# leejeongho3214/LightHand

Hardware: AMD Instinct MI355X
Metric: images/sec/GPU (256×256, bs=64) train+infer; EPE/AUC parity (higher is better)
Workload: dtype bf16; 1 GPU; SimpleBaseline-ResNet50 256x256 training step (fwd + JointsMSELoss + argmax decode + bwd + Adam), batch 64/GPU, 21 joints, random init (seed 9001), hipGraph replay; global_batch=64, parallelism=dp1

## Files before the change

### lighthand_amd/csrc/conv3x3_direct_kernel.h

```cpp
#pragma once
#include "igemm_ring_kernel.h"
#include "igemm_wave_epilogue.h"
#include <stdlib.h>

#pragma clang diagnostic push
#pragma clang diagnostic ignored "-Winline-asm"
__device__ __forceinline__ void d3_lds_dma16(const unsigned char* src, unsigned lds) {
    asm volatile("s_mov_b32 m0, %1\n\ts_nop 0\n\tglobal_load_lds_dwordx4 %0, off" ::"v"(src), "s"(lds) : "memory", "m0");
}
#pragma clang diagnostic pop

template <typename T, int C, bool STATS, bool GATE = false>
__device__ __forceinline__ void conv3x3_direct_body(const IgemmArgs& p, unsigned char* smem, const int b) {
    constexpr int ES = sizeof(T);
    static_assert(ES == 2 && (C == 32 || C == 64), "16-bit element types, 32 or 64 input channels per tap");
    constexpr int BM = 64, TH = 16, TW = 16, PH = TH + 2, PW = TW + 2;
    constexpr int NWAVE = 8;
    constexpr int ROWB = C * ES;
    constexpr int SL = ROWB / 16;
    constexpr int PPI = 1024 / ROWB;
    constexpr int KS = C / 32;
    constexpr int WBYTES = 9 * BM * ROWB;
    constexpr int NPIX = PH * PW;
    constexpr int NPI = (NPIX + PPI - 1) / PPI;
    constexpr int NPW = (NPI + NWAVE - 1) / NWAVE;
    constexpr int PATCH = NPIX * ROWB;
    constexpr int PT = TH / NWAVE;
    constexpr int RS = 64 * ES + 8;
    constexpr int STG = PT * 16 * RS;
    constexpr bool ALIAS = NWAVE * STG <= PATCH;
    constexpr int OFF_PATCH = WBYTES, OFF_STG = WBYTES + 2 * PATCH, OFF_CST = OFF_STG + (ALIAS ? 0 : NWAVE * STG);
    constexpr int NWT = WBYTES / 1024;

    const int tid = threadIdx.x, lane = tid & 63;
    const int wave = __builtin_amdgcn_readfirstlane(tid >> 6);
    const int q = lane >> 4, pl = lane & 15;
    const unsigned lds_base = (unsigned)(size_t)(__attribute__((address_space(3))) unsigned char*)smem;
    const int CB = p.pw_cb, G = p.pw_g;
    const int cblk = (b >> 3) % CB;
// ... 54 lines not shown
        flive = tile < ntile;
        const int tt = flive ? tile : 0;
        const int n = tt / (ty_n * tx_n), rem = tt - n * (ty_n * tx_n);
        fy0 = (rem / tx_n) * TH - 1;
        fx0 = (rem % tx_n) * TW - 1;
        fbase = p.in + n * img_stride;
    };
    auto fetch_piece = [&](int j, int buf) {
        const int iy = fy0 + ppy[j], ix = fx0 + ppx[j];
        const bool ok = flive & ((unsigned)iy < (unsigned)p.hi) & ((unsigned)ix < (unsigned)p.wi);
        const unsigned char* src = ok ? fbase + iy * row_stride + (long)ix * pix_stride + pch[j] : p.zero;
        const unsigned dst = lds_base + OFF_PATCH + buf * PATCH + (NWAVE * j + wave) * 1024;
        if (!(LH_ABL & 4) && ppy[j] >= 0) d3_lds_dma16(src, dst);
    };
    unsigned aoff[KS];
#pragma unroll
    for (int kk = 0; kk < KS; ++kk) aoff[kk] = pl * ROWB + ((((SL == 8 ? 4 * kk : 0) + q) ^ fswz(pl)) << 4);

    float s1[STATS ? 1 : 1][8], s2[STATS ? 1 : 1][8], s3[1][8];
#pragma unroll
    for (int e = 0; e < 8; ++e) s1[0][e] = s2[0][e] = 0.f;
    const float* cst = reinterpret_cast<const float*>(smem + OFF_CST);

    int t = g;
    tile_origin(t);
#pragma unroll
    for (int j = 0; j < NPW; ++j) fetch_piece(j, 0);
    asm volatile("s_waitcnt vmcnt(0)" ::: "memory");
    int buf = 0;
    for (; t < ntile; t += G, buf ^= 1) {
        asm volatile("s_waitcnt lgkmcnt(0)" ::: "memory");
        __builtin_amdgcn_s_barrier();
        asm volatile("" ::: "memory");
        tile_origin(t + G);
        const unsigned char* patch = smem + OFF_PATCH + buf * PATCH;
        f32x4 acc[4][PT];
#pragma unroll
        for (int i = 0; i < 4; ++i)
#pragma unroll
            for (int j = 0; j < PT; ++j) acc[i][j] = f32x4{0.f, 0.f, 0.f, 0.f};
        constexpr int NSTEP = 9 * KS;
        static_assert(NPW <= NSTEP, "one patch piece per MFMA step");
        uint4 A[2][4], B[2][PT];
        auto rd = [&](int step, uint4 (&a)[4], uint4 (&bb)[PT]) {
            const int tap = step / KS, kk = step % KS;
            const int dy = p.dh[tap] + 1, dx = p.dw[tap] + 1;
#pragma unroll
            for (int i = 0; i < 4; ++i) {
                if (LH_ABL & 2) a[i] = uint4{aoff[kk] + i, 3u, 5u, 7u};
                else a[i] = *reinterpret_cast<const uint4*>(smem + tap * (BM * ROWB) + i * 16 * ROWB + aoff[kk]);
            }
#pragma unroll
            for (int j = 0; j < PT; ++j) {
                const int pp = (PT * wave + j + dy) * PW + dx + pl;
                const unsigned off = pp * ROWB + ((((SL == 8 ? 4 * kk : 0) + q) ^ fswz(pp)) << 4);
                if (LH_ABL & 2) bb[j] = uint4{off, 1u, 2u, 3u};
                else bb[j] = *reinterpret_cast<const uint4*>(patch + off);
            }
// ... 9 lines not shown
#pragma unroll
                for (int j = 0; j < PT; ++j) {
                    if (LH_ABL & 1) acc[i][j][0] += __builtin_bit_cast(float, A[step & 1][i].x ^ B[step & 1][j].x);
                    else MmaR<T>::run(A[step & 1][i], B[step & 1][j], acc[i][j]);
                }
            __builtin_amdgcn_sched_barrier(0);
        }
        if (LH_ABL & 8) {
            float z = 0.f;
#pragma unroll
            for (int i = 0; i < 4; ++i)
#pragma unroll
                for (int j = 0; j < PT; ++j) z += acc[i][j][0] + acc[i][j][1] + acc[i][j][2] + acc[i][j][3];
            if (z == 123.456f) p.out[0] = 1;
            asm volatile("s_waitcnt vmcnt(0)" ::: "memory");
            continue;
        }
        if (ALIAS) {
            asm volatile("s_waitcnt lgkmcnt(0)" ::: "memory");
            __builtin_amdgcn_s_barrier();
            asm volatile("" ::: "memory");
        }
        unsigned char* stg = (ALIAS ? smem + OFF_PATCH + buf * PATCH : smem + OFF_STG) + wave * STG;
        const int n = t / (ty_n * tx_n), rem = t - n * (ty_n * tx_n);
        const int oy0 = (rem / tx_n) * TH + PT * wave, ox0 = (rem % tx_n) * TW;
        wave_epilogue<T, BM, PT, STATS, (GATE ? 1 : 0)>(p, acc, stg, cst, cblk, lane, [&](int row) {
            const int y = oy0 + (row >> 4), x = ox0 + (row & 15);
            return (y < H && x < W) ? ((long)n * H + y) * W + x : -1L;
        }, s1, s2, s3);
        asm volatile("s_waitcnt vmcnt(%0)" ::"n"(2 * PT) : "memory");
    }
    if constexpr (STATS) {
        asm volatile("s_waitcnt vmcnt(0)" ::: "memory");
        __syncthreads();
        wave_stats_row<BM, NWAVE>(s1, s2, reinterpret_cast<float*>(smem), p.stats ? p.stats + (long)g * 2 * p.cout : nullptr, cblk, p.cout, tid);
    }
}

template <typename T, int C, bool STATS, bool GATE = false>
__global__ __launch_bounds__(512, 2) void conv3x3_direct_kernel(const IgemmArgs p) {
    extern __shared__ __attribute__((aligned(16))) unsigned char smem[];
    conv3x3_direct_body<T, C, STATS, GATE>(p, smem, blockIdx.x);
}

static inline int lh_d3_lds_bytes(int c) {
    const int patch = 18 * 18 * c * 2, stg = 8 * 2 * 16 * 136;
    return 9 * 64 * c * 2 + 2 * patch + (stg <= patch ? 0 : stg) + 2 * 64 * 4;
}

static inline void lh_d3_grid(int c, int n, int h, int w, int cout, int* G, int* CB) {
    const int cb = (cout + 63) / 64;
    const int occ = lh_d3_lds_bytes(c) <= 80 * 1024 ? 2 : 1;
// ... 33 lines not shown
```

### lighthand_amd/csrc/igemm_epilogue.h

```cpp
#pragma once
#include "common.h"
#include "igemm_args.h"

#ifndef LH_ABL
#define LH_ABL 0
#endif

template <typename T, int BM, int BP, bool HEAD> constexpr int lh_epi_lds_bytes() {
    return BP * (BM * (int)sizeof(T) + 8) + (HEAD ? 32 * (BM * (int)sizeof(T) + 16) : 0) + 3 * BM * 4;
}

template <int BM, int NT>
__device__ __forceinline__ void igemm_epilogue_consts(const IgemmArgs& p, float* cst, int c0, int tid) {
    const int cmax = p.cout - 1;
    for (int c = tid; c < BM; c += NT) {
        const int gc = c0 + c, gk = gc < cmax ? gc : cmax;
        const bool ok = gc < p.cout;
        const float b = p.bias ? p.bias[gk] : 0.f, sc = p.scale ? p.scale[gk] : 1.f, sh = p.scale ? p.shift[gk] : 0.f;
        float bv = (p.bias && ok) ? b : 0.f, sv = 1.f;
        if (p.scale) {
            sv = ok ? sc : 1.f;
            bv = bv * sv + (ok ? sh : 0.f);
        }
        cst[c] = sv;
        cst[BM + c] = bv;
    }
}

template <int NR, int EPC, bool GATE> struct EpilogueGate {
    uint4 xd[NR];
    unsigned gbits[NR];
    float gmean[EPC], ginv[EPC], gsc[EPC], gsh[EPC];
};
template <int NR, int EPC> struct EpilogueGate<NR, EPC, false> {};

template <typename T, int BM, int BP, int WC, int WP, bool GATE = false>
__device__ __forceinline__ void igemm_epilogue(const IgemmArgs& p, unsigned char* smem, f32x4 (&acc)[BM / WC / 16][BP / WP / 16],
                                               int pblk, int cblk, int tid, int lane, int wc, int wp, int hw,
                                               int ooh, int oow, float* stats) {
    constexpr int ES = sizeof(T);
    constexpr int EPC = 16 / ES;
    constexpr int TC = BM / WC, TP = BP / WP;
    constexpr int CT = TC / 16, PT = TP / 16;
    constexpr int RS = BM * ES + 8;
    if (LH_ABL & 8) { if (acc[0][0][0] == 123.456f) p.out[0] = 1; return; }
    if (LH_ABL & 32) {
        float t = 0.f;
#pragma unroll
        for (int i = 0; i < BM / WC / 16; ++i)
#pragma unroll
            for (int j = 0; j < BP / WP / 16; ++j) t += acc[i][j][0] + acc[i][j][1] + acc[i][j][2] + acc[i][j][3];
        if (t == 123.456f) p.out[0] = 1;
        return;
    }
    __syncthreads();
    float* cst = reinterpret_cast<float*>(smem + BP * RS);
    const bool affine = p.bias || p.scale;
    if (affine) {
        igemm_epilogue_consts<BM, 64 * WC * WP>(p, cst, cblk * BM, tid);
        __syncthreads();
    }
    const int q = lane >> 4, pl = lane & 15;
#pragma unroll
    for (int i = 0; i < CT; ++i) {
        const int col = wc * TC + i * 16 + q * 4;
        float4 s4 = float4{1.f, 1.f, 1.f, 1.f}, b4 = float4{0.f, 0.f, 0.f, 0.f};
        if (affine) {
            s4 = *reinterpret_cast<const float4*>(cst + col);
            b4 = *reinterpret_cast<const float4*>(cst + BM + col);
        }
        const float sv[4] = {s4.x, s4.y, s4.z, s4.w}, bv[4] = {b4.x, b4.y, b4.z, b4.w};
#pragma unroll
        for (int j = 0; j < PT; ++j) {
            const int pr = wp * TP + j * 16 + pl;
            T* dst = reinterpret_cast<T*>(smem + pr * RS + col * ES);
            if constexpr (ES == 4) {
                reinterpret_cast<float2*>(dst)[0] = float2{acc[i][j][0] * sv[0] + bv[0], acc[i][j][1] * sv[1] + bv[1]};
                reinterpret_cast<float2*>(dst)[1] = float2{acc[i][j][2] * sv[2] + bv[2], acc[i][j][3] * sv[3] + bv[3]};
            } else {
                union { uint2 u; T e[4]; } pk;
#pragma unroll
                for (int r = 0; r < 4; ++r) pk.e[r] = from_f<T>(acc[i][j][r] * sv[r] + bv[r]);
                *reinterpret_cast<uint2*>(dst) = pk.u;
            }
        }
    }
    __syncthreads();

    constexpr int CH = BM * ES / 16;
    constexpr int NT = 64 * WC * WP;
    constexpr int RPP = NT / CH;
    const int chunk = tid % CH, r0 = tid / CH;
    const int col0 = cblk * BM + chunk * EPC;
    const bool col_ok = col0 < p.cout;
    float s1[EPC], s2[EPC];
#pragma unroll
    for (int e = 0; e < EPC; ++e) s1[e] = s2[e] = 0.f;

    const bool dense = p.osh == 1 && p.osw == 1 && p.OH == p.ho && p.OW == p.wo && ooh == 0 && oow == 0;
    int m = pblk * BP + r0;
    int pn = 0, pa = 0, pb = 0;
    const int qa = RPP / p.wo, step_b = RPP - qa * p.wo, step_n = qa / p.ho, step_a = qa - step_n * p.ho;
    if (!dense) {
        pn = m / hw;
        const int rem = m - pn * hw;
        pa = rem / p.wo;
        pb = rem - pa * p.wo;
    }
    constexpr int NR = BP / RPP;
    static_assert(BP % RPP == 0, "rows per thread");
    int opx[NR];
    uint4 ad[NR];
    unsigned mbits[NR];
    EpilogueGate<NR, EPC, GATE> gt;
    if constexpr (GATE) {
#pragma unroll
        for (int e = 0; e < EPC; ++e) {
            const int gk = col0 + e < p.cout ? col0 + e : p.cout - 1;
            gt.gmean[e] = p.gmean[gk]; gt.ginv[e] = p.ginv[gk];
            gt.gsc[e] = p.gmask ? 0.f : p.gscale[gk]; gt.gsh[e] = p.gmask ? 0.f : p.gshift[gk];
        }
    }
#pragma unroll
    for (int k = 0; k < NR; ++k, m += RPP) {
        int opix = m;
        if (!dense) {
            opix = (pn * p.OH + pa * p.osh + ooh) * p.OW + pb * p.osw + oow;
            pb += step_b; pa += step_a; pn += step_n;
            if (pb >= p.wo) { pb -= p.wo; ++pa; }
            if (pa >= p.ho) { pa -= p.ho; ++pn; }
        }
        opx[k] = (m < p.M && col_ok) ? opix : -1;
        ad[k] = uint4{0u, 0u, 0u, 0u};
        mbits[k] = 0xffu;
        if (p.addend) {
            const bool ok = opx[k] >= 0;
            const long eoff = (long)((unsigned long)(unsigned)(ok ? opx[k] : 0) * (unsigned)p.out_pix_stride) + col0;
            ad[k] = *reinterpret_cast<const uint4*>(ok ? p.addend + eoff * ES : p.zero);
            if (p.addend_mask) mbits[k] = *(ok ? p.addend_mask + eoff / EPC : p.zero);
        }
        if constexpr (GATE) {
            gt.gbits[k] = 0xffu;
            const bool ok = opx[k] >= 0;
            const long eoff = (long)((unsigned long)(unsigned)(ok ? opx[k] : 0) * (unsigned)p.out_pix_stride) + col0;
            gt.xd[k] = *reinterpret_cast<const uint4*>(ok ? p.gx + eoff * ES : p.zero);
            if (p.gmask) gt.gbits[k] = *(ok ? p.gmask + eoff / EPC : p.zero);
        }
    }
#pragma unroll
    for (int k = 0; k < NR; ++k) {
        if (opx[k] < 0) continue;
        const int pr = r0 + k * RPP;
        const long eoff = (long)((unsigned long)(unsigned)opx[k] * (unsigned)p.out_pix_stride) + col0;
        const unsigned char* src = smem + pr * RS + chunk * 16;
        const uint2 lo = *reinterpret_cast<const uint2*>(src);
        const uint2 hi = *reinterpret_cast<const uint2*>(src + 8);
        uint4 u = uint4{lo.x, lo.y, hi.x, hi.y};
        if (p.addend || p.relu) {
            float v[EPC];
            unpack16<T>(u, v);
            if (p.addend) {
                float av[EPC];
                unpack16<T>(ad[k], av);
                if (p.addend_mask) {
#pragma unroll
                    for (int e = 0; e < EPC; ++e) av[e] = ((mbits[k] >> e) & 1u) ? av[e] : 0.f;
                }
#pragma unroll
                for (int e = 0; e < EPC; ++e) v[e] += av[e];
            }
            if (p.relu) {
// ... 133 lines not shown
```

### lighthand_amd/csrc/igemm_pw_kernel.h

```cpp
#pragma once
#include "igemm_ring_kernel.h"
#include "igemm_wave_epilogue.h"
#include <stdlib.h>

template <typename T, int BM, int KC, int PT, bool STATS, int GATE = 0>
__global__ __launch_bounds__(256, 2) void igemm_pw_kernel(const IgemmArgs p) {
    static_assert(!GATE || STATS, "the gate leaves its sums in the statistics row");
    constexpr bool DB = KC <= 256 && !(BM == 256 && KC >= 128) && (2 * PT * (KC / 32) * 4 + (BM / 16) * PT * 4 + (STATS ? (BM / 64) * 16 : 0)) <= 176;
    extern __shared__ __attribute__((aligned(16))) unsigned char smem[];
    constexpr int ES = sizeof(T);
    static_assert(ES == 2, "16-bit element types only");
    constexpr int EPC = 8;
    constexpr int CT = BM / 16;
    constexpr int KS = KC / 32;
    constexpr int NSP = KC / 64;
    constexpr int SPB = BM * 128;
    constexpr int PANEL = NSP * SPB;
    constexpr int SUBW = 64;
    constexpr int NSB = BM / SUBW;
    constexpr int RS = SUBW * ES + 8;
    constexpr int STG = PT * 16 * RS;
    constexpr int CST = PANEL + 4 * STG;
    constexpr int NI = PANEL / 1024;
    static_assert(NI % 4 == 0 && NI / 4 <= 60, "panel fill: instructions per wave");

    const int tid = threadIdx.x, lane = tid & 63;
    const int wave = __builtin_amdgcn_readfirstlane(tid >> 6);
    const int q = lane >> 4, pl = lane & 15;
    const int CB = p.pw_cb, G = p.pw_g;
    const int b = blockIdx.x;
    const int cblk = (b >> 3) % CB;
// ... 61 lines not shown
        }
    };
    int t = g * 4 + wave;
    uint4 B0[PT][KS], B1[DB ? PT : 1][DB ? KS : 1];
    loadB(t, B0);
    asm volatile("s_waitcnt vmcnt(0)" ::: "memory");
    __syncthreads();

    const unsigned aoff0 = pl * 128 + (((0 + q) ^ ((pl >> 1) & 7)) << 4);
    const unsigned aoff1 = pl * 128 + (((4 + q) ^ ((pl >> 1) & 7)) << 4);
    unsigned char* stg = smem + PANEL + wave * STG;
    const float* cst = reinterpret_cast<const float*>(smem + CST);

    float s1[STATS ? NSB : 1][EPC], s2[STATS ? NSB : 1][EPC], s3[GATE == 2 ? NSB : 1][EPC];
#pragma unroll
    for (int i = 0; i < (STATS ? NSB : 1); ++i)
#pragma unroll
        for (int e = 0; e < EPC; ++e) s1[i][e] = s2[i][e] = 0.f;
#pragma unroll
    for (int i = 0; i < (GATE == 2 ? NSB : 1); ++i)
#pragma unroll
        for (int e = 0; e < EPC; ++e) s3[i][e] = 0.f;

    auto tilework = [&](const int t, uint4 (&Bf)[PT][KS], auto&& prefetch) {
        f32x4 acc[CT][PT];
#pragma unroll
        for (int i = 0; i < CT; ++i)
#pragma unroll
            for (int j = 0; j < PT; ++j) acc[i][j] = f32x4{0.f, 0.f, 0.f, 0.f};
        constexpr int NG = KS * (CT / 4);
        uint4 A[2][4];
        auto readA = [&](auto Gc, uint4 (&dst)[4]) {
            constexpr int grp = decltype(Gc)::value;
            constexpr int kk = grp / (CT / 4), i0 = (grp % (CT / 4)) * 4;
#pragma unroll
            for (int u = 0; u < 4; ++u)
                if (LH_ABL & 2) dst[u] = uint4{aoff0 + u, aoff1, 5u, 7u};
                else dst[u] = *reinterpret_cast<const uint4*>(smem + (kk >> 1) * SPB + (i0 + u) * 2048 + ((kk & 1) ? aoff1 : aoff0));
        };
        readA(ic<0>{}, A[0]);
        static_for<0, NG>([&](auto Gc) {
            constexpr int grp = decltype(Gc)::value;
            constexpr int kk = grp / (CT / 4), i0 = (grp % (CT / 4)) * 4;
            if constexpr (grp + 1 < NG) readA(ic<grp + 1>{}, A[(grp + 1) & 1]);
            __builtin_amdgcn_sched_barrier(0);
#pragma unroll
            for (int u = 0; u < 4; ++u)
#pragma unroll
                for (int j = 0; j < PT; ++j) {
                    if (LH_ABL & 1) acc[i0 + u][j][0] += __builtin_bit_cast(float, A[grp & 1][u].x ^ Bf[j][kk].x);
                    else MmaR<T>::run(A[grp & 1][u], Bf[j][kk], acc[i0 + u][j]);
                }
            __builtin_amdgcn_sched_barrier(0);
        });
        prefetch();

        if (LH_ABL & 8) {
            float z = 0.f;
#pragma unroll
            for (int i = 0; i < CT; ++i)
#pragma unroll
                for (int j = 0; j < PT; ++j) z += acc[i][j][0] + acc[i][j][1] + acc[i][j][2] + acc[i][j][3];
            if (z == 123.456f) p.out[0] = 1;
            return;
        }
        const int m0 = t * PT * 16;
        wave_epilogue<T, BM, PT, STATS, GATE>(p, acc, stg, cst, cblk, lane, [&](int row) { const int m = m0 + row; return m < M ? (long)m : -1L; }, s1, s2, s3);
    };
    if constexpr (DB) {
        while (t < ntile) {
            loadB(t + tstride, B1);
            tilework(t, B0, [] {});
            t += tstride;
            if (t >= ntile) break;
            loadB(t + tstride, B0);
            tilework(t, B1, [] {});
            t += tstride;
        }
    } else {
        for (; t < ntile; t += tstride) tilework(t, B0, [&] { loadB(t + tstride, B0); });
    }

    if constexpr (STATS) {
        __syncthreads();
        wave_stats_row<BM, 4>(s1, s2, reinterpret_cast<float*>(smem), p.stats ? p.stats + (long)g * 2 * p.cout : nullptr, cblk, p.cout, tid);
        if constexpr (GATE == 2) {
            __syncthreads();
            wave_stats_row<BM, 4>(s1, s3, reinterpret_cast<float*>(smem), p.stats2 + (long)g * 2 * p.cout, cblk, p.cout, tid);
        }
    }
// ... 35 lines not shown
```

### lighthand_amd/csrc/igemm_ring_kernel.h

```cpp
#pragma once
#include "common.h"
#include "igemm_args.h"
#include "igemm_epilogue.h"
#include "multi.h"

#include <type_traits>

template <typename T> struct MmaR;
template <> struct MmaR<bf16> {
    static __device__ __forceinline__ void run(const uint4& a, const uint4& b, f32x4& c) {
        c = __builtin_amdgcn_mfma_f32_16x16x32_bf16(__builtin_bit_cast(bf16x8, a), __builtin_bit_cast(bf16x8, b), c, 0, 0, 0);
    }
};
template <> struct MmaR<f16> {
    static __device__ __forceinline__ void run(const uint4& a, const uint4& b, f32x4& c) {
        c = __builtin_amdgcn_mfma_f32_16x16x32_f16(__builtin_bit_cast(f16x8, a), __builtin_bit_cast(f16x8, b), c, 0, 0, 0);
    }
};
template <> struct MmaR<float> {
    static __device__ __forceinline__ void run(const uint4& a, const uint4& b, f32x4& c) {
        const f32x4 fa = __builtin_bit_cast(f32x4, a), fb = __builtin_bit_cast(f32x4, b);
        c = __builtin_amdgcn_mfma_f32_16x16x4f32(fa[0], fb[0], c, 0, 0, 0);
        c = __builtin_amdgcn_mfma_f32_16x16x4f32(fa[1], fb[1], c, 0, 0, 0);
        c = __builtin_amdgcn_mfma_f32_16x16x4f32(fa[2], fb[2], c, 0, 0, 0);
// ... 44 lines not shown
    constexpr int L = NW + NX;
    constexpr int KSUB = KB / 64;
    constexpr int NR = PT + CT;
    static_assert((NWAVE == 4 || NWAVE == 8) && D >= 2 && D <= 10 && (KB == 64 || KB == 128) && NW >= 1 && NX >= 1, "bad configuration");

    const int tid = threadIdx.x, lane = tid & 63;
    const int wave = __builtin_amdgcn_readfirstlane(tid >> 6);
    const int wc = wave / WP, wp = wave % WP;
    const int CB = (p.cout + BM - 1) / BM;
    int w = p.xcd ? lh_xcd_remap(bid, nblk) : bid;
    const unsigned char* wgt = p.w;
    int ntaps = p.ntaps, tw = p.tw, dh0 = p.dh0, dhs = p.dhs, dw0 = p.dw0, dws = p.dws, ooh = p.ooh, oow = p.oow;
    float* stats = p.stats;
    if (p.nphase > 1) {
        const int ph = w % p.nphase;
        w /= p.nphase;
        wgt = p.ph_w[ph]; ntaps = p.ph_ntaps[ph]; tw = p.ph_tw[ph];
        dh0 = p.ph_dh0[ph]; dhs = p.ph_dhs[ph]; dw0 = p.ph_dw0[ph]; dws = p.ph_dws[ph];
        ooh = p.ph_ooh[ph]; oow = p.ph_oow[ph];
        if (stats) stats += (long)p.ph_row0[ph] * 2 * p.cout;
    }
    const int pblk = w / CB, cblk = w - pblk * CB;
    const int hw = p.ho * p.wo;

    constexpr unsigned OOR = 0x80000000u;
    const int th = (ntaps + tw - 1) / tw;
    const long ipix = (long)p.in_pix_stride * ES;
    const long shift = ((long)((dh0 < 0 ? -dh0 : dh0) + (dhs < 0 ? -dhs : dhs) * th) * p.wi + (dw0 < 0 ? -dw0 : dw0) + (dws < 0 ? -dws : dws) * tw) * ipix;
    const long img_bytes = (long)p.hi * p.wi * ipix;
    const int m_first = pblk * BP < p.M ? pblk * BP : p.M - 1;
    const int n_first = m_first / hw;
    const long in_off = (long)n_first * img_bytes - shift;
    const long in_rec = (long)p.n * img_bytes - in_off + 16;
    const auto rs_in = __builtin_amdgcn_make_buffer_rsrc((void*)(p.in + in_off), 0, (int)(in_rec < 0x7fffffffL ? in_rec : 0x7fffffffL), 0x00020000);
    const long kpad = p.kpad;
    const long w_off = (long)cblk * BM * ntaps * kpad * ES;
    const auto rs_w = __builtin_amdgcn_make_buffer_rsrc((void*)(wgt + w_off), 0, (int)((long)BM * ntaps * kpad * ES), 0x00020000);
    unsigned pvoff[NX], cvoff[NX];
    unsigned tmask[NX];
    int klim[NX];
    const bool kfull = p.k_run % KSTEP == 0;
#pragma unroll
    for (int j = 0; j < NX; ++j) {
        const int q = NWAVE * j + wave;
        const int g = q / H, lrow = (q % H) * RPI + lane / SL;
        const int c = (lane % SL) ^ ((lrow / (16 / SL)) & (SL - 1));
// ... 52 lines not shown
            ikc = 0; ++itap;
            woff = (int)((long)itap * kpad * ES);
            cdw += dws;
            if (++tj == tw) { tj = 0; cdw = dw0; cdh += dhs; }
            retap = true;
        }
        if (retap || !kfull) {
            const int kb2 = ikc * KSTEP;
#pragma unroll
            for (int j = 0; j < NX; ++j) cvoff[j] = (((tmask[j] >> itap) & 1u) != 0 && kb2 < klim[j]) ? pvoff[j] : OOR;
        }
    };

    f32x4 acc[CT][PT];
#pragma unroll
    for (int i = 0; i < CT; ++i)
#pragma unroll
        for (int j = 0; j < PT; ++j) acc[i][j] = f32x4{0.f, 0.f, 0.f, 0.f};

    const int S = ntaps * p.kspt;
#pragma unroll
    for (int s = 0; s < D - 1; ++s)
        if (issued < S) issue();

    unsigned offA[KSUB], offB[KSUB];
#pragma unroll
    for (int kk = 0; kk < KSUB; ++kk) {
        const int c = 4 * kk + (lane >> 4), r = lane & 15;
        const unsigned foff = r * KB + ((c ^ ((r / (16 / SL)) & (SL - 1))) << 4);
        offA[kk] = lds_base + wc * CT * GB + foff;
        offB[kk] = lds_base + BM * KB + wp * PT * GB + foff;
    }
    auto rd = [](auto Rc, uint4& dst, unsigned base_a, unsigned base_b) {
        constexpr int r = decltype(Rc)::value;
        if constexpr ((LH_ABL & 2) != 0) { dst = uint4{base_a, base_b, base_a, base_b}; return; }
        if constexpr (r < PT) asm volatile("ds_read_b128 %0, %1 offset:%2" : "=v"(dst) : "v"(base_b), "n"(r * GB));
        else asm volatile("ds_read_b128 %0, %1 offset:%2" : "=v"(dst) : "v"(base_a), "n"((r - PT) * GB));
    };
    auto step_at = [&](const unsigned ca, const unsigned cb) {
        uint4 F[NR];
        static_for<0, NR>([&](auto r) { rd(r, F[decltype(r)::value], ca, cb); });
        static_for<0, CT>([&](auto Ic) {
            constexpr int i = decltype(Ic)::value;
            __builtin_amdgcn_sched_barrier(0);
            asm volatile("s_waitcnt lgkmcnt(%0)" ::"n"(CT - 1 - i) : "memory");
            __builtin_amdgcn_sched_barrier(0);
// ... 4 lines not shown
    };
    auto step = [&](auto KKc, unsigned so) { step_at(offA[decltype(KKc)::value] + so, offB[decltype(KKc)::value] + so); };

    const bool late = NWAVE == 8 && KSUB == 2 && wave >= NWAVE / 2;
    int cslot = 0;
    for (int s = 0; s < S; ++s) {
        wait_stages<L, D - 2>(issued - 1 - s);
        __builtin_amdgcn_s_barrier();
        const unsigned so = cslot * STAGE;
        if (++cslot == D) cslot = 0;
        if (!late && issued < S) issue();
        step(ic<0>{}, so);
        if constexpr (KSUB == 2) {
            if (late && issued < S) issue();
            step(ic<1>{}, so);
        }
    }
    if constexpr (BM == 256 && BP == 256 && sizeof(T) == 2 && !GATE) {
        if (p.head_w) {
            igemm_epilogue_head<T, BM, BP, WC, WP, MmaR<T>>(p, smem, acc, pblk, tid, lane, wave, wc, wp, hw, ooh, oow);
            return;
        }
    }
    igemm_epilogue<T, BM, BP, WC, WP, GATE>(p, smem, acc, pblk, cblk, tid, lane, wc, wp, hw, ooh, oow, stats);
#endif
}

template <int BM, int BP, int WC, int WP> constexpr int ring_waves_per_simd() { return 2; }

template <typename T, int BM, int BP, int WC, int WP, int D, int KB>
__global__ __launch_bounds__(64 * WC * WP, (ring_waves_per_simd<BM, BP, WC, WP>())) void igemm_ring_kernel(const IgemmArgs p) {
    extern __shared__ __attribute__((aligned(16))) unsigned char smem[];
    igemm_ring_body<T, BM, BP, WC, WP, D, KB>(p, smem, blockIdx.x, gridDim.x);
}

template <typename T, int BM, int BP, int WC, int WP, int D, int KB>
__global__ __launch_bounds__(64 * WC * WP, (ring_waves_per_simd<BM, BP, WC, WP>())) void igemm_ring_gated_kernel(const IgemmArgs p) {
    extern __shared__ __attribute__((aligned(16))) unsigned char smem[];
    igemm_ring_body<T, BM, BP, WC, WP, D, KB, true>(p, smem, blockIdx.x, gridDim.x);
}

template <typename T, int BM, int BP, int WC, int WP, int D, int KB>
__global__ __launch_bounds__(64 * WC * WP, 2) void igemm_ring_multi_kernel(const LhMulti<IgemmArgs> m) {
    extern __shared__ __attribute__((aligned(16))) unsigned char smem[];
    int bid, nblk;
    const int i = lh_multi_pick(m, bid, nblk);
    igemm_ring_body<T, BM, BP, WC, WP, D, KB>(m.a[i], smem, bid, nblk);
// ... 50 lines not shown
```

### lighthand_amd/csrc/igemm_wave_epilogue.h

```cpp
#pragma once
#include "common.h"
#include "igemm_args.h"

#ifndef LH_ABL
#define LH_ABL 0
#endif

template <typename T, int BM, int PT, bool STATS, int GATE = 0, typename PixFn, int NS, int NS3>
__device__ __forceinline__ void wave_epilogue(const IgemmArgs& p, f32x4 (&acc)[BM / 16][PT], unsigned char* stg, const float* cst,
                                              const int cblk, const int lane, PixFn&& pix, float (&s1)[NS][8], float (&s2)[NS][8],
                                              float (&s3)[NS3][8]) {
    constexpr int ES = sizeof(T), EPC = 8, SUBW = 64, NSB = BM / SUBW, RS = SUBW * ES + 8;
    const int q = lane >> 4, pl = lane & 15;
    const int rrow = lane >> 3, rch = lane & 7;
#pragma unroll
    for (int sb = 0; sb < NSB; ++sb) {
        __builtin_amdgcn_sched_barrier(0);
#pragma unroll
        for (int it = 0; it < 4; ++it) {
            const int i = sb * 4 + it;
            const int col = i * 16 + q * 4;
            const float4 sv = GATE ? float4{1.f, 1.f, 1.f, 1.f} : *reinterpret_cast<const float4*>(cst + col);
            const float4 bv = GATE ? float4{0.f, 0.f, 0.f, 0.f} : *reinterpret_cast<const float4*>(cst + BM + col);
#pragma unroll
            for (int j = 0; j < PT; ++j) {
                union { uint2 u; T e[4]; } pk;
                pk.e[0] = from_f<T>(acc[i][j][0] * sv.x + bv.x);
                pk.e[1] = from_f<T>(acc[i][j][1] * sv.y + bv.y);
                pk.e[2] = from_f<T>(acc[i][j][2] * sv.z + bv.z);
// ... 94 lines not shown
                    for (int e = 0; e < EPC; ++e) { s1[sb][e] += g[e]; s2[sb][e] += g[e] * (xv[e] - gmean[e]) * ginv[e]; }
                    if constexpr (GATE == 2) {
                        float x2[EPC];
                        unpack16<T>(xd2[k], x2);
#pragma unroll
                        for (int e = 0; e < EPC; ++e) s3[sb][e] += g[e] * (x2[e] - gmean2[e]) * ginv2[e];
                    }
                }
                u = pack16<T>(g);
            } else if constexpr (STATS) {
                if (opix[k] >= 0) {
                    float fv[EPC];
                    unpack16<T>(u, fv);
#pragma unroll
                    for (int e = 0; e < EPC; ++e) { s1[sb][e] += fv[e]; s2[sb][e] += fv[e] * fv[e]; }
                }
            }
            unsigned char* dst = opix[k] >= 0 ? p.out + (opix[k] * p.out_pix_stride + col0) * ES : p.dump + lane * 16;
            if (!(LH_ABL & 16) || u.x == 0x12345678u) *reinterpret_cast<uint4*>(dst) = u;
        }
    }
}

template <int BM, int NWAVE, int NS>
__device__ __forceinline__ void wave_stats_row(float (&s1)[NS][8], float (&s2)[NS][8], float* red, float* stats_row, const int cblk,
                                               const int cout, const int tid) {
    constexpr int EPC = 8, SUBW = 64, NSB = BM / SUBW;
    const int lane = tid & 63, wave = tid >> 6;
#pragma unroll
    for (int sb = 0; sb < NSB; ++sb)
#pragma unroll
        for (int e = 0; e < EPC; ++e) {
            float a = s1[sb][e], c = s2[sb][e];
#pragma unroll
            for (int o = 8; o < 64; o <<= 1) { a += __shfl_xor(a, o); c += __shfl_xor(c, o); }
            if (lane < 8) {
                red[(wave * 2 + 0) * BM + sb * SUBW + lane * EPC + e] = a;
                red[(wave * 2 + 1) * BM + sb * SUBW + lane * EPC + e] = c;
            }
        }
    __syncthreads();
    if (stats_row) {
        for (int i = tid; i < 2 * BM; i += 64 * NWAVE) {
            const int which = i / BM, col = i - which * BM;
            float a = red[(0 * 2 + which) * BM + col];
#pragma unroll
// ... 7 lines not shown
```

Before: 7673 images/s.

## Prefetch gated epilogue side inputs before MFMA main loop in conv kernels

For the gated (backward BN/ReLU gate) variants of the direct 3x3, pointwise and ring implicit-GEMM kernels, the epilogue's global reads (gate input, masks, addend) are issued before the MFMA main loop, or during the previous sub-block, instead of after accumulation. The aim is to hide their memory latency behind the matrix math. A per-shape table decides which pointwise configurations use the early path. The cost is more live registers across the main loop, which may lower occupancy or cause spills.

```diff
diff --git a/lighthand_amd/csrc/conv3x3_direct_kernel.h b/lighthand_amd/csrc/conv3x3_direct_kernel.h
--- a/lighthand_amd/csrc/conv3x3_direct_kernel.h
+++ b/lighthand_amd/csrc/conv3x3_direct_kernel.h
@@ -15,6 +15,7 @@
     constexpr int ES = sizeof(T);
     static_assert(ES == 2 && (C == 32 || C == 64), "16-bit element types, 32 or 64 input channels per tap");
     constexpr int BM = 64, TH = 16, TW = 16, PH = TH + 2, PW = TW + 2;
+    constexpr int PF = GATE ? 2 : 0;
     constexpr int NWAVE = 8;
     constexpr int ROWB = C * ES;
     constexpr int SL = ROWB / 16;
@@ -115,6 +116,14 @@
     for (int e = 0; e < 8; ++e) s1[0][e] = s2[0][e] = 0.f;
     const float* cst = reinterpret_cast<const float*>(smem + OFF_CST);
 
+    auto tile_pix = [&](const int t) {
+        const int n = t / (ty_n * tx_n), rem = t - n * (ty_n * tx_n);
+        const int oy0 = (rem / tx_n) * TH + PT * wave, ox0 = (rem % tx_n) * TW;
+        return [=](int row) {
+            const int y = oy0 + (row >> 4), x = ox0 + (row & 15);
+            return (y < H && x < W) ? ((long)n * H + y) * W + x : -1L;
+        };
+    };
     int t = g;
     tile_origin(t);
 #pragma unroll
@@ -127,6 +136,8 @@
         asm volatile("" ::: "memory");
         tile_origin(t + G);
         const unsigned char* patch = smem + OFF_PATCH + buf * PATCH;
+        std::conditional_t<PF != 0, WaveEpilogueReads<PT, (GATE ? 1 : 0)>, NoReads> er;
+        if constexpr (PF == 2) wave_epilogue_request<T, BM, PT, (GATE ? 1 : 0)>(p, er, cblk * BM + (lane & 7) * 8, lane >> 3, tile_pix(t));
         f32x4 acc[4][PT];
 #pragma unroll
         for (int i = 0; i < 4; ++i)
@@ -182,12 +193,16 @@
             asm volatile("" ::: "memory");
         }
         unsigned char* stg = (ALIAS ? smem + OFF_PATCH + buf * PATCH : smem + OFF_STG) + wave * STG;
-        const int n = t / (ty_n * tx_n), rem = t - n * (ty_n * tx_n);
-        const int oy0 = (rem / tx_n) * TH + PT * wave, ox0 = (rem % tx_n) * TW;
-        wave_epilogue<T, BM, PT, STATS, (GATE ? 1 : 0)>(p, acc, stg, cst, cblk, lane, [&](int row) {
-            const int y = oy0 + (row >> 4), x = ox0 + (row & 15);
-            return (y < H && x < W) ? ((long)n * H + y) * W + x : -1L;
-        }, s1, s2, s3);
+        if constexpr (PF != 0) {
+            wave_epilogue_ahead<T, BM, PT, STATS, (GATE ? 1 : 0), PF>(p, acc, stg, cst, cblk, lane, tile_pix(t), s1, s2, s3, er);
+        } else {
+            const int n = t / (ty_n * tx_n), rem = t - n * (ty_n * tx_n);
+            const int oy0 = (rem / tx_n) * TH + PT * wave, ox0 = (rem % tx_n) * TW;
+            wave_epilogue<T, BM, PT, STATS, (GATE ? 1 : 0)>(p, acc, stg, cst, cblk, lane, [&](int row) {
+                const int y = oy0 + (row >> 4), x = ox0 + (row & 15);
+                return (y < H && x < W) ? ((long)n * H + y) * W + x : -1L;
+            }, s1, s2, s3);
+        }
         asm volatile("s_waitcnt vmcnt(%0)" ::"n"(2 * PT) : "memory");
     }
     if constexpr (STATS) {
diff --git a/lighthand_amd/csrc/igemm_epilogue.h b/lighthand_amd/csrc/igemm_epilogue.h
--- a/lighthand_amd/csrc/igemm_epilogue.h
+++ b/lighthand_amd/csrc/igemm_epilogue.h
@@ -34,69 +34,26 @@
 };
 template <int NR, int EPC> struct EpilogueGate<NR, EPC, false> {};
 
-template <typename T, int BM, int BP, int WC, int WP, bool GATE = false>
-__device__ __forceinline__ void igemm_epilogue(const IgemmArgs& p, unsigned char* smem, f32x4 (&acc)[BM / WC / 16][BP / WP / 16],
-                                               int pblk, int cblk, int tid, int lane, int wc, int wp, int hw,
-                                               int ooh, int oow, float* stats) {
+template <typename T, int BM, int BP, int WC, int WP, bool GATE> struct EpiloguePass1 {
+    static constexpr int EPC = 16 / (int)sizeof(T);
+    static constexpr int CH = BM * (int)sizeof(T) / 16;
+    static constexpr int RPP = 64 * WC * WP / CH;
+    static constexpr int NR = BP / RPP;
+    static_assert(BP % RPP == 0, "rows per thread");
+    static constexpr bool EARLY = GATE && NR <= 4;
+    int opx[NR];
+    uint4 ad[NR];
+    unsigned mbits[NR];
+    EpilogueGate<NR, EPC, GATE> gt;
+};
+
+template <typename T, int BM, int BP, int WC, int WP, bool GATE>
+__device__ __forceinline__ void igemm_epilogue_pass1(const IgemmArgs& p, EpiloguePass1<T, BM, BP, WC, WP, GATE>& __restrict__ e, int pblk, int r0, int col0,
+                                                     int hw, int ooh, int oow) {
     constexpr int ES = sizeof(T);
     constexpr int EPC = 16 / ES;
-    constexpr int TC = BM / WC, TP = BP / WP;
-    constexpr int CT = TC / 16, PT = TP / 16;
-    constexpr int RS = BM * ES + 8;
-    if (LH_ABL & 8) { if (acc[0][0][0] == 123.456f) p.out[0] = 1; return; }
-    if (LH_ABL & 32) {
-        float t = 0.f;
-#pragma unroll
-        for (int i = 0; i < BM / WC / 16; ++i)
-#pragma unroll
-            for (int j = 0; j < BP / WP / 16; ++j) t += acc[i][j][0] + acc[i][j][1] + acc[i][j][2] + acc[i][j][3];
-        if (t == 123.456f) p.out[0] = 1;
-        return;
-    }
-    __syncthreads();
-    float* cst = reinterpret_cast<float*>(smem + BP * RS);
-    const bool affine = p.bias || p.scale;
-    if (affine) {
-        igemm_epilogue_consts<BM, 64 * WC * WP>(p, cst, cblk * BM, tid);
-        __syncthreads();
-    }
-    const int q = lane >> 4, pl = lane & 15;
-#pragma unroll
-    for (int i = 0; i < CT; ++i) {
-        const int col = wc * TC + i * 16 + q * 4;
-        float4 s4 = float4{1.f, 1.f, 1.f, 1.f}, b4 = float4{0.f, 0.f, 0.f, 0.f};
-        if (affine) {
-            s4 = *reinterpret_cast<const float4*>(cst + col);
-            b4 = *reinterpret_cast<const float4*>(cst + BM + col);
-        }
-        const float sv[4] = {s4.x, s4.y, s4.z, s4.w}, bv[4] = {b4.x, b4.y, b4.z, b4.w};
-#pragma unroll
-        for (int j = 0; j < PT; ++j) {
-            const int pr = wp * TP + j * 16 + pl;
-            T* dst = reinterpret_cast<T*>(smem + pr * RS + col * ES);
-            if constexpr (ES == 4) {
-                reinterpret_cast<float2*>(dst)[0] = float2{acc[i][j][0] * sv[0] + bv[0], acc[i][j][1] * sv[1] + bv[1]};
-                reinterpret_cast<float2*>(dst)[1] = float2{acc[i][j][2] * sv[2] + bv[2], acc[i][j][3] * sv[3] + bv[3]};
-            } else {
-                union { uint2 u; T e[4]; } pk;
-#pragma unroll
-                for (int r = 0; r < 4; ++r) pk.e[r] = from_f<T>(acc[i][j][r] * sv[r] + bv[r]);
-                *reinterpret_cast<uint2*>(dst) = pk.u;
-            }
-        }
-    }
-    __syncthreads();
-
-    constexpr int CH = BM * ES / 16;
-    constexpr int NT = 64 * WC * WP;
-    constexpr int RPP = NT / CH;
-    const int chunk = tid % CH, r0 = tid / CH;
-    const int col0 = cblk * BM + chunk * EPC;
+    constexpr int RPP = EpiloguePass1<T, BM, BP, WC, WP, GATE>::RPP, NR = EpiloguePass1<T, BM, BP, WC, WP, GATE>::NR;
     const bool col_ok = col0 < p.cout;
-    float s1[EPC], s2[EPC];
-#pragma unroll
-    for (int e = 0; e < EPC; ++e) s1[e] = s2[e] = 0.f;
-
     const bool dense = p.osh == 1 && p.osw == 1 && p.OH == p.ho && p.OW == p.wo && ooh == 0 && oow == 0;
     int m = pblk * BP + r0;
     int pn = 0, pa = 0, pb = 0;
@@ -107,18 +64,12 @@
         pa = rem / p.wo;
         pb = rem - pa * p.wo;
     }
-    constexpr int NR = BP / RPP;
-    static_assert(BP % RPP == 0, "rows per thread");
-    int opx[NR];
-    uint4 ad[NR];
-    unsigned mbits[NR];
-    EpilogueGate<NR, EPC, GATE> gt;
     if constexpr (GATE) {
 #pragma unroll
-        for (int e = 0; e < EPC; ++e) {
-            const int gk = col0 + e < p.cout ? col0 + e : p.cout - 1;
-            gt.gmean[e] = p.gmean[gk]; gt.ginv[e] = p.ginv[gk];
-            gt.gsc[e] = p.gmask ? 0.f : p.gscale[gk]; gt.gsh[e] = p.gmask ? 0.f : p.gshift[gk];
+        for (int x = 0; x < EPC; ++x) {
+            const int gk = col0 + x < p.cout ? col0 + x : p.cout - 1;
+            e.gt.gmean[x] = p.gmean[gk]; e.gt.ginv[x] = p.ginv[gk];
+            e.gt.gsc[x] = p.gmask ? 0.f : p.gscale[gk]; e.gt.gsh[x] = p.gmask ? 0.f : p.gshift[gk];
         }
     }
 #pragma unroll
@@ -130,23 +81,96 @@
             if (pb >= p.wo) { pb -= p.wo; ++pa; }
             if (pa >= p.ho) { pa -= p.ho; ++pn; }
         }
-        opx[k] = (m < p.M && col_ok) ? opix : -1;
-        ad[k] = uint4{0u, 0u, 0u, 0u};
-        mbits[k] = 0xffu;
+        e.opx[k] = (m < p.M && col_ok) ? opix : -1;
+        e.ad[k] = uint4{0u, 0u, 0u, 0u};
+        e.mbits[k] = 0xffu;
         if (p.addend) {
-            const bool ok = opx[k] >= 0;
-            const long eoff = (long)((unsigned long)(unsigned)(ok ? opx[k] : 0) * (unsigned)p.out_pix_stride) + col0;
-            ad[k] = *reinterpret_cast<const uint4*>(ok ? p.addend + eoff * ES : p.zero);
-            if (p.addend_mask) mbits[k] = *(ok ? p.addend_mask + eoff / EPC : p.zero);
+            const bool ok = e.opx[k] >= 0;
+            const long eoff = (long)((unsigned long)(unsigned)(ok ? e.opx[k] : 0) * (unsigned)p.out_pix_stride) + col0;
+            e.ad[k] = *reinterpret_cast<const uint4*>(ok ? p.addend + eoff * ES : p.zero);
+            if (p.addend_mask) e.mbits[k] = *(ok ? p.addend_mask + eoff / EPC : p.zero);
         }
         if constexpr (GATE) {
-            gt.gbits[k] = 0xffu;
-            const bool ok = opx[k] >= 0;
-            const long eoff = (long)((unsigned long)(unsigned)(ok ? opx[k] : 0) * (unsigned)p.out_pix_stride) + col0;
-            gt.xd[k] = *reinterpret_cast<const uint4*>(ok ? p.gx + eoff * ES : p.zero);
-            if (p.gmask) gt.gbits[k] = *(ok ? p.gmask + eoff / EPC : p.zero);
-        }
-    }
+            e.gt.gbits[k] = 0xffu;
+            const bool ok = e.opx[k] >= 0;
+            const long eoff = (long)((unsigned long)(unsigned)(ok ? e.opx[k] : 0) * (unsigned)p.out_pix_stride) + col0;
+            e.gt.xd[k] = *reinterpret_cast<const uint4*>(ok ? p.gx + eoff * ES : p.zero);
+            if (p.gmask) e.gt.gbits[k] = *(ok ? p.gmask + eoff / EPC : p.zero);
+        }
+    }
+}
+
+template <typename T, int BM, int BP, int WC, int WP, bool GATE = false>
+__device__ __forceinline__ void igemm_epilogue(const IgemmArgs& p, unsigned char* smem, f32x4 (&acc)[BM / WC / 16][BP / WP / 16],
+                                               int pblk, int cblk, int tid, int lane, int wc, int wp, int hw,
+                                               int ooh, int oow, float* stats, EpiloguePass1<T, BM, BP, WC, WP, GATE>& e1) {
+    constexpr int ES = sizeof(T);
+    constexpr int EPC = 16 / ES;
+    constexpr int TC = BM / WC, TP = BP / WP;
+    constexpr int CT = TC / 16, PT = TP / 16;
+    constexpr int RS = BM * ES + 8;
+    if (LH_ABL & 8) { if (acc[0][0][0] == 123.456f) p.out[0] = 1; return; }
+    if (LH_ABL & 32) {
+        float t = 0.f;
+#pragma unroll
+        for (int i = 0; i < BM / WC / 16; ++i)
+#pragma unroll
+            for (int j = 0; j < BP / WP / 16; ++j) t += acc[i][j][0] + acc[i][j][1] + acc[i][j][2] + acc[i][j][3];
+        if (t == 123.456f) p.out[0] = 1;
+        return;
+    }
+    __syncthreads();
+    float* cst = reinterpret_cast<float*>(smem + BP * RS);
+    const bool affine = p.bias || p.scale;
+    if (affine) {
+        igemm_epilogue_consts<BM, 64 * WC * WP>(p, cst, cblk * BM, tid);
+        __syncthreads();
+    }
+    const int q = lane >> 4, pl = lane & 15;
+#pragma unroll
+    for (int i = 0; i < CT; ++i) {
+        const int col = wc * TC + i * 16 + q * 4;
+        float4 s4 = float4{1.f, 1.f, 1.f, 1.f}, b4 = float4{0.f, 0.f, 0.f, 0.f};
+        if (affine) {
+            s4 = *reinterpret_cast<const float4*>(cst + col);
+            b4 = *reinterpret_cast<const float4*>(cst + BM + col);
+        }
+        const float sv[4] = {s4.x, s4.y, s4.z, s4.w}, bv[4] = {b4.x, b4.y, b4.z, b4.w};
+#pragma unroll
+        for (int j = 0; j < PT; ++j) {
+            const int pr = wp * TP + j * 16 + pl;
+            T* dst = reinterpret_cast<T*>(smem + pr * RS + col * ES);
+            if constexpr (ES == 4) {
+                reinterpret_cast<float2*>(dst)[0] = float2{acc[i][j][0] * sv[0] + bv[0], acc[i][j][1] * sv[1] + bv[1]};
+                reinterpret_cast<float2*>(dst)[1] = float2{acc[i][j][2] * sv[2] + bv[2], acc[i][j][3] * sv[3] + bv[3]};
+            } else {
+                union { uint2 u; T e[4]; } pk;
+#pragma unroll
+                for (int r = 0; r < 4; ++r) pk.e[r] = from_f<T>(acc[i][j][r] * sv[r] + bv[r]);
+                *reinterpret_cast<uint2*>(dst) = pk.u;
+            }
+        }
+    }
+    __syncthreads();
+
+    constexpr int CH = BM * ES / 16;
+    constexpr int NT = 64 * WC * WP;
+    constexpr int RPP = NT / CH;
+    const int chunk = tid % CH, r0 = tid / CH;
+    const int col0 = cblk * BM + chunk * EPC;
+    float s1[EPC], s2[EPC];
+#pragma unroll
+    for (int e = 0; e < EPC; ++e) s1[e] = s2[e] = 0.f;
+
+    constexpr int NR = BP / RPP;
+    using Pass1 = EpiloguePass1<T, BM, BP, WC, WP, GATE>;
+    Pass1 late;
+    if constexpr (!Pass1::EARLY) igemm_epilogue_pass1<T, BM, BP, WC, WP, GATE>(p, late, pblk, r0, col0, hw, ooh, oow);
+    const Pass1& ps = [&]() -> const Pass1& { if constexpr (Pass1::EARLY) return e1; else return late; }();
+    const int (&opx)[NR] = ps.opx;
+    const uint4 (&ad)[NR] = ps.ad;
+    const unsigned (&mbits)[NR] = ps.mbits;
+    const EpilogueGate<NR, EPC, GATE>& gt = ps.gt;
 #pragma unroll
     for (int k = 0; k < NR; ++k) {
         if (opx[k] < 0) continue;
diff --git a/lighthand_amd/csrc/igemm_pw_kernel.h b/lighthand_amd/csrc/igemm_pw_kernel.h
--- a/lighthand_amd/csrc/igemm_pw_kernel.h
+++ b/lighthand_amd/csrc/igemm_pw_kernel.h
@@ -3,10 +3,22 @@
 #include "igemm_wave_epilogue.h"
 #include <stdlib.h>
 
+template <int BM, int KC, int PT, bool STATS, int GATE> constexpr int pw_epilogue_prefetch() {
+    if (!GATE) return 0;
+    if (BM == 128 && KC == 256 && PT == 1) return 2;
+    if (BM == 256 && KC == 64 && GATE == 1) return 2;
+    if (BM == 64 && KC == 128 && PT == 2) return 2;
+    if (BM == 64 && KC == 64 && PT == 2 && GATE == 2) return 2;
+    if (BM == 64 && KC == 512) return 2;
+    if (BM == 128 && KC == 512 && GATE == 1) return 2;
+    return 0;
+}
+
 template <typename T, int BM, int KC, int PT, bool STATS, int GATE = 0>
 __global__ __launch_bounds__(256, 2) void igemm_pw_kernel(const IgemmArgs p) {
     static_assert(!GATE || STATS, "the gate leaves its sums in the statistics row");
     constexpr bool DB = KC <= 256 && !(BM == 256 && KC >= 128) && (2 * PT * (KC / 32) * 4 + (BM / 16) * PT * 4 + (STATS ? (BM / 64) * 16 : 0)) <= 176;
+    constexpr int PF = pw_epilogue_prefetch<BM, KC, PT, STATS, GATE>();
     extern __shared__ __attribute__((aligned(16))) unsigned char smem[];
     constexpr int ES = sizeof(T);
     static_assert(ES == 2, "16-bit element types only");
@@ -114,7 +126,13 @@
 #pragma unroll
         for (int e = 0; e < EPC; ++e) s3[i][e] = 0.f;
 
+    auto tile_pix = [M](const int t) {
+        const int m0 = t * PT * 16;
+        return [m0, M](int row) { const int m = m0 + row; return m < M ? (long)m : -1L; };
+    };
     auto tilework = [&](const int t, uint4 (&Bf)[PT][KS], auto&& prefetch) {
+        std::conditional_t<PF != 0, WaveEpilogueReads<PT, GATE>, NoReads> er;
+        if constexpr (PF == 2) wave_epilogue_request<T, BM, PT, GATE>(p, er, cblk * BM + (lane & 7) * EPC, lane >> 3, tile_pix(t));
         f32x4 acc[CT][PT];
 #pragma unroll
         for (int i = 0; i < CT; ++i)
@@ -156,8 +174,12 @@
             if (z == 123.456f) p.out[0] = 1;
             return;
         }
-        const int m0 = t * PT * 16;
-        wave_epilogue<T, BM, PT, STATS, GATE>(p, acc, stg, cst, cblk, lane, [&](int row) { const int m = m0 + row; return m < M ? (long)m : -1L; }, s1, s2, s3);
+        if constexpr (PF != 0) {
+            wave_epilogue_ahead<T, BM, PT, STATS, GATE, PF>(p, acc, stg, cst, cblk, lane, tile_pix(t), s1, s2, s3, er);
+        } else {
+            const int m0 = t * PT * 16;
+            wave_epilogue<T, BM, PT, STATS, GATE>(p, acc, stg, cst, cblk, lane, [&](int row) { const int m = m0 + row; return m < M ? (long)m : -1L; }, s1, s2, s3);
+        }
     };
     if constexpr (DB) {
         while (t < ntile) {
diff --git a/lighthand_amd/csrc/igemm_ring_kernel.h b/lighthand_amd/csrc/igemm_ring_kernel.h
--- a/lighthand_amd/csrc/igemm_ring_kernel.h
+++ b/lighthand_amd/csrc/igemm_ring_kernel.h
@@ -90,6 +90,9 @@
     }
     const int pblk = w / CB, cblk = w - pblk * CB;
     const int hw = p.ho * p.wo;
+
+    using Pass1 = EpiloguePass1<T, BM, BP, WC, WP, GATE>;
+    Pass1 e1;
 
     constexpr unsigned OOR = 0x80000000u;
     const int th = (ntaps + tw - 1) / tw;
@@ -188,6 +191,7 @@
 #pragma unroll
     for (int s = 0; s < D - 1; ++s)
         if (issued < S) issue();
+    if constexpr (Pass1::EARLY) igemm_epilogue_pass1<T, BM, BP, WC, WP, GATE>(p, e1, pblk, tid / Pass1::CH, cblk * BM + tid % Pass1::CH * EPC, hw, ooh, oow);
 
     unsigned offA[KSUB], offB[KSUB];
 #pragma unroll
@@ -238,7 +242,7 @@
             return;
         }
     }
-    igemm_epilogue<T, BM, BP, WC, WP, GATE>(p, smem, acc, pblk, cblk, tid, lane, wc, wp, hw, ooh, oow, stats);
+    igemm_epilogue<T, BM, BP, WC, WP, GATE>(p, smem, acc, pblk, cblk, tid, lane, wc, wp, hw, ooh, oow, stats, e1);
 #endif
 }
 
diff --git a/lighthand_amd/csrc/igemm_wave_epilogue.h b/lighthand_amd/csrc/igemm_wave_epilogue.h
--- a/lighthand_amd/csrc/igemm_wave_epilogue.h
+++ b/lighthand_amd/csrc/igemm_wave_epilogue.h
@@ -5,6 +5,43 @@
 #ifndef LH_ABL
 #define LH_ABL 0
 #endif
+
+template <int PT, int GATE> struct WaveEpilogueReads {
+    static constexpr int NP = PT * 2;
+    uint4 ad[NP];
+    unsigned mb[NP];
+    long opix[NP];
+    uint4 xd[GATE ? NP : 1];
+    uint4 xd2[GATE == 2 ? NP : 1];
+    unsigned gm[GATE ? NP : 1];
+};
+
+struct NoReads {};
+
+template <typename T, int BM, int PT, int GATE, typename PixFn>
+__device__ __forceinline__ void wave_epilogue_request(const IgemmArgs& p, WaveEpilogueReads<PT, GATE>& __restrict__ r, const int col0, const int rrow,
+                                                      PixFn&& pix) {
+    constexpr int ES = sizeof(T), EPC = 8, NP = PT * 2;
+    const bool col_ok = col0 < p.cout;
+#pragma unroll
+    for (int k = 0; k < NP; ++k) {
+        r.opix[k] = col_ok ? pix(k * 8 + rrow) : -1L;
+        r.ad[k] = uint4{0u, 0u, 0u, 0u};
+        r.mb[k] = 0xffu;
+        if (p.addend) {
+            const long eoff = r.opix[k] * p.out_pix_stride + col0;
+            r.ad[k] = *reinterpret_cast<const uint4*>(r.opix[k] >= 0 ? p.addend + eoff * ES : p.zero);
+            if (p.addend_mask) r.mb[k] = *(r.opix[k] >= 0 ? p.addend_mask + eoff / EPC : p.zero);
+        }
+        if constexpr (GATE) {
+            const long eoff = r.opix[k] * p.out_pix_stride + col0;
+            r.xd[k] = *reinterpret_cast<const uint4*>(r.opix[k] >= 0 ? p.gx + eoff * ES : p.zero);
+            r.gm[k] = 0xffu;
+            if (p.gmask) r.gm[k] = *(r.opix[k] >= 0 ? p.gmask + eoff / EPC : p.zero);
+            if constexpr (GATE == 2) r.xd2[k] = *reinterpret_cast<const uint4*>(r.opix[k] >= 0 ? p.gx2 + eoff * ES : p.zero);
+        }
+    }
+}
 
 template <typename T, int BM, int PT, bool STATS, int GATE = 0, typename PixFn, int NS, int NS3>
 __device__ __forceinline__ void wave_epilogue(const IgemmArgs& p, f32x4 (&acc)[BM / 16][PT], unsigned char* stg, const float* cst,
@@ -145,6 +182,134 @@
     }
 }
 
+template <typename T, int BM, int PT, bool STATS, int GATE, int PF, typename PixFn, int NS, int NS3>
+__device__ __forceinline__ void wave_epilogue_ahead(const IgemmArgs& p, f32x4 (&acc)[BM / 16][PT], unsigned char* stg, const float* cst,
+                                              const int cblk, const int lane, PixFn&& pix, float (&s1)[NS][8], float (&s2)[NS][8],
+                                              float (&s3)[NS3][8], WaveEpilogueReads<PT, GATE>& first) {
+    static_assert(PF == 1 || PF == 2, "PF = 0 is wave_epilogue itself");
+    constexpr int ES = sizeof(T), EPC = 8, SUBW = 64, NSB = BM / SUBW, RS = SUBW * ES + 8;
+    const int q = lane >> 4, pl = lane & 15;
+    const int rrow = lane >> 3, rch = lane & 7;
+    WaveEpilogueReads<PT, GATE> ahead[2];
+#pragma unroll
+    for (int sb = 0; sb < NSB; ++sb) {
+        __builtin_amdgcn_sched_barrier(0);
+        if (sb + 1 < NSB) {
+            wave_epilogue_request<T, BM, PT, GATE>(p, ahead[(sb + 1) & 1], cblk * BM + (sb + 1) * SUBW + rch * EPC, rrow, pix);
+            __builtin_amdgcn_sched_barrier(0);
+        }
+#pragma unroll
+        for (int it = 0; it < 4; ++it) {
+            const int i = sb * 4 + it;
+            const int col = i * 16 + q * 4;
+            const float4 sv = GATE ? float4{1.f, 1.f, 1.f, 1.f} : *reinterpret_cast<const float4*>(cst + col);
+            const float4 bv = GATE ? float4{0.f, 0.f, 0.f, 0.f} : *reinterpret_cast<const float4*>(cst + BM + col);
+#pragma unroll
+            for (int j = 0; j < PT; ++j) {
+                union { uint2 u; T e[4]; } pk;
+                pk.e[0] = from_f<T>(acc[i][j][0] * sv.x + bv.x);
+                pk.e[1] = from_f<T>(acc[i][j][1] * sv.y + bv.y);
+                pk.e[2] = from_f<T>(acc[i][j][2] * sv.z + bv.z);
+                pk.e[3] = from_f<T>(acc[i][j][3] * sv.w + bv.w);
+                *reinterpret_cast<uint2*>(stg + (j * 16 + pl) * RS + (it * 16 + q * 4) * ES) = pk.u;
+            }
+        }
+        const int col0 = cblk * BM + sb * SUBW + rch * EPC;
+        constexpr int NP = PT * 2;
+        float gmean[EPC], ginv[EPC], gsc[EPC], gsh[EPC], gmean2[EPC], ginv2[EPC];
+        if constexpr (GATE) {
+            const int cc = sb * SUBW + rch * EPC;
+#pragma unroll
+            for (int h = 0; h < 2; ++h) {
+                const float4 a = *reinterpret_cast<const float4*>(cst + cc + 4 * h), b = *reinterpret_cast<const float4*>(cst + BM + cc + 4 * h);
+                float4 c = float4{0.f, 0.f, 0.f, 0.f}, d = c;
+                if constexpr (GATE != 2) {
+                    c = *reinterpret_cast<const float4*>(cst + 2 * BM + cc + 4 * h);
+                    d = *reinterpret_cast<const float4*>(cst + 3 * BM + cc + 4 * h);
+                }
+                gmean[4 * h] = a.x; gmean[4 * h + 1] = a.y; gmean[4 * h + 2] = a.z; gmean[4 * h + 3] = a.w;
+                ginv[4 * h] = b.x; ginv[4 * h + 1] = b.y; ginv[4 * h + 2] = b.z; ginv[4 * h + 3] = b.w;
+                if constexpr (GATE != 2) {
+                    gsc[4 * h] = c.x; gsc[4 * h + 1] = c.y; gsc[4 * h + 2] = c.z; gsc[4 * h + 3] = c.w;
+                    gsh[4 * h] = d.x; gsh[4 * h + 1] = d.y; gsh[4 * h + 2] = d.z; gsh[4 * h + 3] = d.w;
+                }
+                if constexpr (GATE == 2) {
+                    const float4 a2 = *reinterpret_cast<const float4*>(cst + 4 * BM + cc + 4 * h), b2 = *reinterpret_cast<const float4*>(cst + 5 * BM + cc + 4 * h);
+                    gmean2[4 * h] = a2.x; gmean2[4 * h + 1] = a2.y; gmean2[4 * h + 2] = a2.z; gmean2[4 * h + 3] = a2.w;
+                    ginv2[4 * h] = b2.x; ginv2[4 * h + 1] = b2.y; ginv2[4 * h + 2] = b2.z; ginv2[4 * h + 3] = b2.w;
+                }
+            }
+        }
+        if constexpr (PF == 1) { if (sb == 0) wave_epilogue_request<T, BM, PT, GATE>(p, first, col0, rrow, pix); }
+        const WaveEpilogueReads<PT, GATE>& rd = sb == 0 ? first : ahead[sb & 1];
+        const uint4 (&ad)[NP] = rd.ad;
+        const unsigned (&mb)[NP] = rd.mb;
+        const long (&opix)[NP] = rd.opix;
+        const uint4 (&xd)[GATE ? NP : 1] = rd.xd;
+        const uint4 (&xd2)[GATE == 2 ? NP : 1] = rd.xd2;
+        const unsigned (&gm)[GATE ? NP : 1] = rd.gm;
+#pragma unroll
+        for (int k = 0; k < NP; ++k) {
+            const int row = k * 8 + rrow;
+            const unsigned char* src = stg + row * RS + rch * 16;
+            const uint2 lo = *reinterpret_cast<const uint2*>(src);
+            const uint2 hi = *reinterpret_cast<const uint2*>(src + 8);
+            uint4 u = uint4{lo.x, lo.y, hi.x, hi.y};
+            if (p.addend || p.relu) {
+                float v[EPC];
+                unpack16<T>(u, v);
+                if (p.addend) {
+                    float av[EPC];
+                    unpack16<T>(ad[k], av);
+                    if (p.addend_mask) {
+#pragma unroll
+                        for (int e = 0; e < EPC; ++e) av[e] = ((mb[k] >> e) & 1u) ? av[e] : 0.f;
+                    }
+#pragma unroll
+                    for (int e = 0; e < EPC; ++e) v[e] += av[e];
+                }
+                if (p.relu) {
+#pragma unroll
+                    for (int e = 0; e < EPC; ++e) v[e] = fmaxf(v[e], 0.f);
+                }
+                u = pack16<T>(v);
+            }
+            if constexpr (GATE) {
+                float g[EPC], xv[EPC];
+                unpack16<T>(u, g);
+                unpack16<T>(xd[k], xv);
+                if (GATE == 2 || p.gmask) {
+#pragma unroll
+                    for (int e = 0; e < EPC; ++e) g[e] = ((gm[k] >> e) & 1u) ? g[e] : 0.f;
+                } else if constexpr (GATE != 2) {
+#pragma unroll
+                    for (int e = 0; e < EPC; ++e) g[e] = (xv[e] * gsc[e] + gsh[e]) > 0.f ? g[e] : 0.f;
+                }
+                if (opix[k] >= 0) {
+#pragma unroll
+                    for (int e = 0; e < EPC; ++e) { s1[sb][e] += g[e]; s2[sb][e] += g[e] * (xv[e] - gmean[e]) * ginv[e]; }
+                    if constexpr (GATE == 2) {
+                        float x2[EPC];
+                        unpack16<T>(xd2[k], x2);
+#pragma unroll
+                        for (int e = 0; e < EPC; ++e) s3[sb][e] += g[e] * (x2[e] - gmean2[e]) * ginv2[e];
+                    }
+                }
+                u = pack16<T>(g);
+            } else if constexpr (STATS) {
+                if (opix[k] >= 0) {
+                    float fv[EPC];
+                    unpack16<T>(u, fv);
+#pragma unroll
+                    for (int e = 0; e < EPC; ++e) { s1[sb][e] += fv[e]; s2[sb][e] += fv[e] * fv[e]; }
+                }
+            }
+            unsigned char* dst = opix[k] >= 0 ? p.out + (opix[k] * p.out_pix_stride + col0) * ES : p.dump + lane * 16;
+            if (!(LH_ABL & 16) || u.x == 0x12345678u) *reinterpret_cast<uint4*>(dst) = u;
+        }
+    }
+}
+
 template <int BM, int NWAVE, int NS>
 __device__ __forceinline__ void wave_stats_row(float (&s1)[NS][8], float (&s2)[NS][8], float* red, float* stats_row, const int cblk,
                                                const int cout, const int tid) {
```

After: 7653 images/s. About the same (-0.3%).
